# drscotthawley/signaltrain

Measured on AMD Instinct MI355X. Metric: audio-frames/sec (train step) comp_4c 8192-sample windows @ 1/2/4/8 GPUs, higher is better.
Workload: dtype f32; 1 GPU; comp_4c synthetic, 8192-sample windows, batch 256/GPU, fp32 (BASELINE configs[1]); window=8192, frames_per_window=25, global_batch=256, parallelism=dp1

## Files before the change

### signaltrain_amd/csrc/st_api.hip

```cpp
#include <hip/hip_runtime.h>
#include <stdarg.h>
#include <stdio.h>
#include <string.h>
#include <math.h>
#include <mutex>
#include <set>
#include <type_traits>
#include <utility>
#include "st_common.h"
#include "st_gemm.h"
#include "st_gemm_planes.h"
#include "st_gemm_tn.h"
#include "st_gemm16.h"
#include "st_misc.h"
#include "st_ae.h"
#include "st_ae_wide.h"
#include "st_ae_split.h"
#include "st_ae32.h"
#include "st_dp.h"
#include "st_feed.h"
#include "st_feed_files.h"
#include "st_feed_live.h"
#include "st_feed_stream.h"
#include "st_predict.h"
// ... 119 lines not shown
    ST_TRY(check_dims(d));
    L->total = param_offsets(d, L->offs);
    L->n_stft = L->offs[4];
    L->PG = (int)(L->offs[22] - L->offs[4]);
    for (int l = 0; l < 9; ++l) {
        L->go.w[l] = (int)(L->offs[4 + 2 * l] - L->offs[4]);
        L->go.b[l] = (int)(L->offs[5 + 2 * l] - L->offs[4]);
    }
    L->KP = st_kp_of(d->F);
    return ST_OK;
}

static int num_cus()
{
    static int n = 0;
    if (!n) { int dev = 0; (void)hipGetDevice(&dev); hipDeviceProp_t p; if (hipGetDeviceProperties(&p, dev) == hipSuccess) n = p.multiProcessorCount; if (n <= 0) n = 256; }
    return n;
}
extern "C" int st_set_debug(int v) { return v == 0 ? ST_OK : st_fail(ST_ERR_ARG, "st_set_debug(%d): the product library has no run-time ablations (build with -DST_*_ABLATE=bits)", v); }
static int g_dp_inline = 1;
static int g_ae_save = 1;
static int g_ae_split = -1;
static int g_ae32 = 1;
static int g_pl_bf16 = 0;
static int g_wg_split = 0;
static int g_pl_dgrad = 0;
static int g_pl_shape = 3;
static int g_g16 = 1;
static int g_g16_dma = 0;
static int g_nt128 = 1;
static int g_tn128 = 1;
static int g_tn_fm = 3;
static int g_g16_crop = 15;
static int g_frs_nt = 1;
static int g_xt = 0;
static const int NORM_E_PARTIALS = 32;
static const int NORM_E_MAX = 4096;
static int g_wide_direct = 1;
static int g_an_bk = 32;
static int g_bk = 16;
static int g_wg_mode = 0;
#define ST_TUNING_LIST(X) X(g_ae_split, -1) X(g_ae_save, 1) X(g_dp_inline, 1) X(g_pl_bf16, 0) X(g_wg_split, 0) X(g_pl_dgrad, 0) X(g_pl_shape, 3) X(g_g16, 1) X(g_g16_dma, 0) \
    X(g_nt128, 1) X(g_tn128, 1) X(g_frs_nt, 1) X(g_xt, 0) X(g_an_bk, 32) X(g_bk, 16) X(g_wg_mode, 0) X(g_ae32, 1) X(g_wide_direct, 1) X(g_tn_fm, 3) X(g_g16_crop, 15)
static const struct { int first, count; int* var; int value; int* also; } k_tuning_codes[] = {
    {16, 1, &g_an_bk, 16, &g_bk}, {32, 1, &g_an_bk, 32, &g_bk},
    {100, 1, &g_wg_mode, 0, nullptr}, {102, 1, &g_wg_mode, 2, nullptr},
    {7000, 2, &g_xt, 0, nullptr},
    {8000, 2, &g_ae_split, 0, nullptr}, {8002, 1, &g_ae_split, -1, nullptr},
    {8100, 2, &g_ae32, 0, nullptr},
    {8200, 3, &g_ae_save, 0, nullptr},
    {8300, 2, &g_dp_inline, 0, nullptr},
    {9000, 2, &g_frs_nt, 0, nullptr},
    {9100, 1, &g_pl_shape, 0, nullptr}, {9103, 1, &g_pl_shape, 3, nullptr},
    {9200, 2, &g_pl_dgrad, 0, nullptr},
    {9300, 2, &g_wg_split, 0, nullptr},
    {9400, 2, &g_pl_bf16, 0, nullptr},
    {9500, 2, &g_tn128, 0, nullptr}, {9580, 1, &g_tn128, 2, nullptr}, {9581, 1, &g_tn128, 1, nullptr},
    {9582, 1, &g_tn128, 3, nullptr},
    {9540, 4, &g_tn_fm, 0, nullptr},
    {9560, 16, &g_g16_crop, 0, nullptr},
    {9600, 2, &g_g16, 0, nullptr},
    {9690, 4, &g_g16_dma, 0, nullptr},
    {9950, 2, &g_nt128, 0, nullptr},
    {9970, 2, &g_wide_direct, 0, nullptr},
};
extern "C" int st_set_tuning(int code)
{
    for (const auto& t : k_tuning_codes)
        if (code >= t.first && code < t.first + t.count) { *t.var = t.value + (code - t.first); if (t.also) *t.also = *t.var; return ST_OK; }
    return st_fail(ST_ERR_ARG, "st_set_tuning(%d): no such code", code);
}
extern "C" int st_get_tuning(int* out, int n)
{
    int i = 0;
#define X(v_, d_) if (out && i < n) out[i] = v_; ++i;
    ST_TUNING_LIST(X)
#undef X
    return i;
}
extern "C" int st_tuning_defaults(int* out, int n)
{
    int i = 0;
#define X(v_, d_) if (out && i < n) out[i] = d_; ++i;
    ST_TUNING_LIST(X)
#undef X
    return i;
}
extern "C" int st_reset_tuning(void)
{
#define X(v_, d_) v_ = d_;
    ST_TUNING_LIST(X)
#undef X
    return ST_OK;
}
static inline int gemm_ht(int prec) { return (prec == ST_PREC_BF16 || prec == ST_PREC_BF16_ALL) ? 1 : ((prec == ST_PREC_F16 || prec == ST_PREC_F16_ALL) ? 2 : (prec == ST_PREC_F32X3 ? 3 : 0)); }
static inline int ae_ht(int prec) { return prec == ST_PREC_BF16_ALL ? 1 : (prec == ST_PREC_F16_ALL ? 2 : 0); }
static inline float loss_scale_of(const st_dims* d) { return d->loss_scale > 0.f ? d->loss_scale : 1.0f; }
static inline float reg_scale_of(const st_dims* d) { return (float)(2e-5 / 10.0) / ((float)d->B * (float)d->OT * (float)d->F); }
static inline float reg_coef_of(const st_dims* d) { return loss_scale_of(d) * (float)(2e-5 / 10.0) / ((float)d->B * (float)d->OT * (float)d->F); }
static inline float expfac_of(const st_dims* d) { return (float)(7.0 / d->F); }
static int ensure_dyn_lds(const void* fn, const char* name)
{
    static std::mutex mu; static std::set<std::pair<int, const void*>> done;
    int dev = 0; (void)hipGetDevice(&dev);
    std::lock_guard<std::mutex> lk(mu);
    if (done.count({dev, fn})) return ST_OK;
// ... 272 lines not shown
}

static stg::RowMap synth_live(const st_dims* d) { return stg::live_frames(d->OT, d->H, d->N, d->N, d->y); }
static int synth_live_rows(const st_dims* d) { return synth_live(d).rows(d->B); }

static double synth_crop_fraction(const st_dims* d)
{
    const stg::RowMap ms = synth_live(d);
    long live = 0;
    for (int t = ms.t_lo; t < ms.t_lo + ms.Tv; ++t) { int lo, hi; stg::ntw_live_taps(t, t, d->H, d->N, d->N, d->y, lo, hi); live += hi - lo; }
    return 1.0 - (double)live / ((double)ms.Tv * (double)d->N);
}
static inline bool fm_div_exact(int R, int B) { return R >= 0 && B >= 1 && (unsigned long long)(unsigned)R * (unsigned long long)(unsigned)B < (1ull << 32); }
extern "C" int st_fm_div_exact(int R, int B) { return fm_div_exact(R, B) ? 1 : 0; }
static bool use_nt128(const st_dims* d, int M, int Nc, int ncus = 0)
{
    if (!(g_nt128 && gemm_ht(d->prec) == 0 && d->N % 32 == 0 && (M + 127) / 128 <= 255 && fm_div_exact(M, d->B))) return false;
    if (ncus <= 0) ncus = num_cus();
    return ((M + 127) / 128) * ((Nc + 127) / 128) * 2 <= ncus || synth_crop_fraction(d) >= 0.10;
}
enum { GEMM_ANALYSIS = 0, GEMM_FRAMES = 1, GEMM_DGRAD = 2 };
enum { SGP_PADDED = 1,
       SGP_G16 = 2,
       SGP_SFOLDT = 4 };
enum { GF_FP32 = 0,
       GF_HALF = 1,
       GF_PLANES = 2,
       GF_G16 = 3 };
enum { GK_SMALL = 0,
       GK_NT128 = 1,
       GK_PLANES = 2,
       GK_NT16 = 3, GK_NT256 = 4 };
static bool use_planes(const st_dims* d) { return (gemm_ht(d->prec) == 3 || (gemm_ht(d->prec) == 1 && g_pl_bf16)) && d->N % 16 == 0 && st_kp_of(d->F) % 16 == 0; }
static int planes_of(const st_dims* d) { return gemm_ht(d->prec) == 3 ? 3 : 1; }
template <class F> static inline auto with_planes(int pl, F&& f) { return pl == 1 ? f(ic<1>{}) : f(ic<3>{}); }
static bool use_g16(const st_dims* d)
{
    const int ht = gemm_ht(d->prec);
    return g_g16 && (ht == 1 || ht == 2) && !g_pl_bf16 && d->N % 128 == 0 && num_cus() > 0;
}
static int stft_family(const st_dims* d, int which, int flags)
{
    if (flags & SGP_PADDED) {
        if ((flags & SGP_G16) && use_g16(d)) return GF_G16;
        if (use_planes(d) && (which != GEMM_DGRAD || g_pl_dgrad)) return GF_PLANES;
    }
    return gemm_ht(d->prec) == 0 ? GF_FP32 : GF_HALF;
}
struct GemmOps { const float *A, *B, *B2; const unsigned short *A16, *B16, *Bpl; float in_scale; };
struct GemmPlan {
    const st_dims* d; GemmOps o;
    int which, flags, family, form;
    int waves, bk, xt;
    bool transposed;
    stg::RowMap live;
    int R, M, Nc, K, ns;
    size_t slab;
    bool frame_major; int crop;
    stg::NTWork wk;
};
static GemmPlan stft_plan(const st_dims* d, int which, int flags, const GemmOps& o, int ncus = 0)
{
    const int KP = st_kp_of(d->F), N = d->N;
    const bool padded = (flags & SGP_PADDED) != 0;
    GemmPlan p; p.d = d; p.o = o; p.which = which; p.flags = flags;
    p.live = which == GEMM_ANALYSIS ? stg::live_frames(d->T, d->H, N, N, d->L)
                                    : synth_live(d);
    p.R = p.M = p.live.rows(d->B);
    p.Nc = which == GEMM_ANALYSIS ? 2 * d->F : which == GEMM_FRAMES ? N : KP; p.K = which == GEMM_FRAMES ? KP : N;
    const SynthTile t = which == GEMM_ANALYSIS ? SynthTile{4, 1} : synth_tile(p.R);
    p.waves = t.waves; p.ns = t.ns; p.slab = which == GEMM_ANALYSIS ? 0 : (size_t)d->B * d->OT * p.Nc;
    p.family = stft_family(d, which, flags);
    p.bk = p.xt = 0; p.transposed = false; p.frame_major = false; p.crop = 0; p.wk.n = 0;
    if (p.family == GF_G16) {
        const int dma = which == GEMM_ANALYSIS ? 1 : which == GEMM_DGRAD ? 2 : 0;
        p.form = ((g_g16_dma & dma) && N % 64 == 0 && N / 64 >= p.ns) ? GK_NT256 : GK_NT16; p.waves = 0;
        const bool crop = which == GEMM_FRAMES ? (g_g16_crop & 1) != 0 : which == GEMM_DGRAD && (g_g16_crop & 2) && !(g_g16_dma & 2);
        if (crop && fm_div_exact(p.R, d->B)) { p.frame_major = true; p.crop = which; }
    } else if (p.family == GF_PLANES) {
        p.form = GK_PLANES;
        if (which == GEMM_ANALYSIS && planes_of(d) == 3 && g_pl_shape == 3) p.waves = 8;
    } else {
        p.form = GK_SMALL;
        p.transposed = which == GEMM_FRAMES && (flags & SGP_SFOLDT) && g_frs_nt;
        const int cus = ncus > 0 ? ncus : num_cus();
        if ((which == GEMM_FRAMES ? p.transposed : which == GEMM_DGRAD && padded) && use_nt128(d, p.R, p.Nc, cus) &&
            (which == GEMM_FRAMES ? stg::ntw_frames(p.wk, p.live, d->B, d->H, N, N, d->y, KP, p.ns, cus)
                                  : stg::ntw_dgrad(p.wk, p.live, d->B, d->H, N, N, d->y, d->F, KP, p.ns, cus))) {
            p.form = GK_NT128; p.waves = 0; p.frame_major = true; p.crop = which;
        } else {
            p.wk.n = 0;
            if (p.family == GF_FP32) { p.bk = (which == GEMM_ANALYSIS && padded) ? g_an_bk : g_bk; p.xt = g_xt ? 1 : 0; }
        }
    }
    return p;
}
struct GemmOut { float *re, *im, *mag, *phs; const PolarWide* pw; float* C; };
static GemmOut slabs_at(float* C) { return GemmOut{nullptr, nullptr, nullptr, nullptr, nullptr, C}; }
static int stft_gemm(const GemmPlan& p, const GemmOut& out, void* stream)
{
    const st_dims* d = p.d; const GemmOps& o = p.o; hipStream_t s = st_stream(stream);
    const int KP = st_kp_of(d->F), N = d->N, R = p.R;
    const stg::RowMap rows = p.frame_major ? stg::frame_major(p.live, d->B) : p.live;
    auto g16 = [&](const stg::Rows16& ra, const stg::Rows16& rb, const auto& ep, const stg::Crop16* cr) {
        return with_ht16(gemm_ht(d->prec), [&](auto HT) {
            return p.form == GK_NT256 ? stg::launch16_nt256<HT()>(ra, rb, ep, p.M, p.Nc, p.K, p.ns, s) : stg::launch16_nt<HT()>(ra, rb, ep, p.M, p.Nc, p.K, p.ns, s, cr); }); };
    if (p.which == GEMM_ANALYSIS) {
        stg::PolarStore ep{out.re, out.im, out.mag, out.phs, R, d->F, rows};
        polar_wide_set(ep, out.pw);
        if (p.family == GF_G16)
            ST_TRY(g16(stg::rows16(o.A16, (unsigned)(d->L + 2 * N), (unsigned)d->H, p.live, R), stg::rows16_plain(o.B16, (unsigned)N, 2 * d->F), ep, nullptr));
        else if (!(p.flags & SGP_PADDED)) {
            stg::FramedNT<false> al{o.A, d->L, d->H, N, R, N, o.in_scale, p.live};
            ST_TRY(small_gemm<4>(d->prec, p.bk, p.xt != 0, al, stg::AnalysisW{o.B, o.B2, d->F, N}, ep, p.M, p.Nc, p.K, p.ns, s));
        } else {
            stg::FramedNT<true> al{o.A, d->L, d->H, N, R, N, 1.0f, p.live};
            if (p.family == GF_PLANES) {
                stg::ChunkP bl{o.Bpl, 2 * d->F};
                ST_TRY((planes_of(d) == 1 ? stg::launch_planes<4, 1>(al, bl, ep, p.M, p.Nc, p.K, p.ns, s) :
                        p.waves == 8 ? stg::launch_planes<8, 3>(al, bl, ep, p.M, p.Nc, p.K, p.ns, s) : stg::launch_planes<4, 3>(al, bl, ep, p.M, p.Nc, p.K, p.ns, s)));
            } else ST_TRY(small_gemm<4>(d->prec, p.bk, p.xt != 0, al, stg::AnalysisW{o.B, o.B2, d->F, N}, ep, p.M, p.Nc, p.K, p.ns, s));
        }
        ST_LAUNCHED("analysis_fwd");
        return ST_OK;
    }
    const bool frames = p.which == GEMM_FRAMES;
    const unsigned s_win = frames ? (unsigned)(d->OT * KP) : (unsigned)(d->y + 2 * N), s_frm = frames ? (unsigned)KP : (unsigned)d->H;
    auto small = [&](const auto& al, const auto& bl) {
        const stg::StoreC ep{out.C, R, p.Nc, p.Nc, p.slab, rows};
        return p.waves == 4 ? small_gemm<4>(d->prec, p.bk, p.xt != 0, al, bl, ep, p.M, p.Nc, p.K, p.ns, s) : small_gemm<2>(d->prec, p.bk, p.xt != 0, al, bl, ep, p.M, p.Nc, p.K, p.ns, s); };
    auto planes = [&](const auto& al) {
        const stg::StoreC ep{out.C, R, p.Nc, p.Nc, p.slab, rows}; const stg::ChunkP bl{o.Bpl, p.Nc};
        return with_planes(planes_of(d), [&](auto PL) {
            return p.waves == 4 ? stg::launch_planes<4, PL()>(al, bl, ep, p.M, p.Nc, p.K, p.ns, s) : stg::launch_planes<2, PL()>(al, bl, ep, p.M, p.Nc, p.K, p.ns, s); }); };
    if (p.family == GF_G16) {
        const stg::Rows16 ra = p.frame_major ? stg::rows16_frame_major(o.A16, s_win, s_frm, p.live, d->B, R) : stg::rows16(o.A16, s_win, s_frm, p.live, R);
        const stg::Crop16 cr{p.crop, d->B, d->H, N, N, d->y, p.live.t_lo, R, 1};
        ST_TRY(g16(ra, stg::rows16_plain(o.B16, (unsigned)p.K, p.Nc), stg::StoreC{out.C, R, p.Nc, p.Nc, p.slab, rows}, &cr));
    } else if (p.form == GK_NT128) {
        const stg::NTRows ra = stg::ntrows_frame_major(o.A, s_win, s_frm, p.live, d->B, R);
        const stg::NTRows rb = frames ? stg::NTRows{o.B2, (unsigned)KP, 0u, 0u, 1, 0, N} :
                               p.wk.col_h ? stg::NTRows{o.B, (unsigned)((KP / 2) * N), (unsigned)N, stg::rowmap_magic(d->F - 1), d->F - 1, 0, 2 * (d->F - 1)}
                                          : stg::NTRows{o.B, (unsigned)N, 0u, 0u, 1, 0, KP};
        ST_TRY(stg::launch_nt128(ra, rb, stg::StoreSlab{out.C, R, p.Nc, p.Nc, p.slab, rows}, p.wk, s));
    } else if (frames) {
        const stg::PlainNT al{o.A, R, KP, KP, p.live};
        if (p.family == GF_PLANES) ST_TRY(planes(al));
        else if (p.transposed) ST_TRY(small(al, stg::PlainNT{o.B2, N, KP, KP, stg::all_frames(1)}));
        else ST_TRY(small(al, stg::PlainTN{o.B, KP, N, N, stg::all_frames(1)}));
    } else {
        const stg::PlainNT bl{o.B, KP, N, N, stg::all_frames(1)};
        if (!(p.flags & SGP_PADDED)) ST_TRY(small(stg::FramedNT<false>{o.A, d->y, d->H, N, R, N, 1.0f, p.live}, bl));
        else {
            const stg::FramedNT<true> al{o.A, d->y, d->H, N, R, N, 1.0f, p.live};
            if (p.family == GF_PLANES) ST_TRY(planes(al)); else ST_TRY(small(al, bl));
        }
    }
    ST_LAUNCHED(frames ? "synthesis_frames" : "synthesis_dgrad");
    return ST_OK;
}
extern "C" int st_analysis_fwd(const st_dims* d, const float* x, const float* Wr, const float* Wi, float in_scale,
                               float* re, float* im, float* mag, float* phs, void* stream)
{
    ST_TRY(check_dims(d)); ST_REQ(x && Wr && Wi, "st_analysis_fwd: null input");
    const GemmPlan p = stft_plan(d, GEMM_ANALYSIS, 0, GemmOps{x, Wr, Wi, nullptr, nullptr, nullptr, in_scale});
    ST_TRY(stft_gemm(p, GemmOut{re, im, mag, phs, nullptr, nullptr}, stream));
    if (p.live.Tv < d->T) {
        hipLaunchKernelGGL(stm::zero_dead_frames_kernel, dim3(d->B * (d->T - p.live.Tv)), dim3(256), 0, st_stream(stream),
                           re, im, mag, phs, d->T, d->F, p.live.t_lo, p.live.Tv);
        ST_LAUNCHED("zero_dead_frames");
    }
    return ST_OK;
}
extern "C" int st_synthesis_frames(const st_dims* d, const float* AA, const float* Sfold, float* frs, void* stream)
// ... 1947 lines not shown
```

### signaltrain_amd/csrc/st_gemm.h

```cpp
#pragma once
#include "st_common.h"

static int ensure_dyn_lds(const void* fn, const char* name);
namespace stg {

constexpr int BK = 32;
constexpr int BN = 96;
constexpr int NJ = BN / 32;
constexpr int PK = BK + 4;

struct RowMap {
    int Tv, t_lo, T; unsigned magic;
    int fm;
    __host__ __device__ int rows(int B) const { return B * Tv; }
    __device__ void split(int r, int& b, int& t) const {
        if (fm) {
            const int q = magic ? (int)__umulhi((unsigned)r, magic) : r;
            b = r - (int)__umul24((unsigned)q, (unsigned)fm);
            t = t_lo + q;
            return;
        }
        b = magic ? (int)__umulhi((unsigned)r, magic) : r;
        t = t_lo + (r - (int)__umul24((unsigned)b, (unsigned)Tv));
    }
    __device__ int full(int r) const { int b, t; split(r, b, t); return (int)__umul24((unsigned)b, (unsigned)T) + t; }
};
static inline unsigned rowmap_magic(int Tv) { return Tv > 1 ? (unsigned)(((unsigned long long)1 << 32) / (unsigned)Tv) + 1u : 0u; }
static inline RowMap live_frames(int T, int H, int N, int pad, int Ls)
{
    int lo = 0, hi = T - 1;
    while (lo < T && H * lo - pad + N <= 0) ++lo;
    while (hi >= lo && H * hi - pad >= Ls) --hi;
    RowMap m; m.t_lo = lo; m.Tv = hi - lo + 1; m.T = T; m.fm = 0;
    if (m.Tv <= 0) { m.Tv = T; m.t_lo = 0; }
    m.magic = rowmap_magic(m.Tv);
    return m;
}
static inline RowMap all_frames(int T) { RowMap m; m.Tv = T; m.t_lo = 0; m.T = T; m.fm = 0; m.magic = rowmap_magic(T); return m; }
static inline RowMap frame_major(RowMap m, int B) { m.fm = B; m.magic = B > 1 ? rowmap_magic(B) : 0u; return m; }

__device__ __forceinline__ float4 ldg128(const float* __restrict__ base, const unsigned elem)
{
    return *reinterpret_cast<const float4*>(reinterpret_cast<const char*>(base) + (size_t)(elem << 2));
}

struct Src { const float* p; bool ok; };

struct TNParams { const float* base; unsigned magic, S1, S2; int Tv, t_lo, clampR, klim, collim; };

struct RowState {
    const float* p;
    unsigned o;
    int lo, hi;
};

template <bool PADDED>
struct FramedNT {
    static constexpr bool kTN = false;
    static constexpr bool kCheck = !PADDED;
    static constexpr bool kOff = true;
    const float* sig; int Ls, H, pad, R, Kw; float scale; RowMap map;
    __device__ const float* dummy() const { return sig; }
    __device__ RowState row_state(int r) const {
        RowState s; s.p = sig; s.o = 0; s.lo = 0; s.hi = 0;
        if (PADDED) {
            int b, t; map.split(r < R ? r : 0, b, t);
            s.o = __umul24((unsigned)b, (unsigned)(Ls + 2 * pad)) + __umul24((unsigned)H, (unsigned)t);
            s.p = sig + s.o;
            s.hi = Kw;
        } else if (r < R) {
            int b, t; map.split(r, b, t);
            const int start = H * t - pad;
            s.o = __umul24((unsigned)b, (unsigned)Ls) + (unsigned)start;
            s.p = sig + (size_t)b * Ls + start;
            s.lo = start < 0 ? -start : 0;
            s.hi = (Ls - start) < Kw ? (Ls - start) : Kw;
            if (s.hi < s.lo) s.hi = s.lo;
        }
        return s;
    }
    __device__ Src src(const RowState& s, int k) const { return Src{s.p + k, PADDED || (k >= s.lo && k < s.hi)}; }
    __device__ float4 post(float4 v) const {
        if (!PADDED) { v.x *= scale; v.y *= scale; v.z *= scale; v.w *= scale; }
        return v;
    }
};

template <bool PADDED>
struct FramedTN {
    static constexpr bool kTN = true;
    static constexpr bool kCheck = !PADDED;
    static constexpr bool kOff = true;
    const float* sig; int Ls, H, pad, R, Kw; float scale; RowMap map;
    __device__ const float* dummy() const { return sig; }
    __device__ Src src(int r, int n) const {
        if (PADDED) {
            int b, t; map.split(r < R ? r : 0, b, t);
            return Src{sig + (size_t)b * (Ls + 2 * pad) + H * t + n, true};
        }
        Src s{sig, false};
        if (r < R && n < Kw) {
            int b, t; map.split(r, b, t);
            const int pos = H * t - pad + n;
            s.ok = pos >= 0 && pos < Ls;
            s.p = sig + (size_t)b * Ls + pos;
        }
        return s;
    }
    __device__ unsigned off(int r, int n, bool& ok) const {
        int b, t;
        map.split(r < R ? r : 0, b, t);
        if (PADDED) {
            ok = true;
            return __umul24((unsigned)b, (unsigned)(Ls + 2 * pad)) + __umul24((unsigned)H, (unsigned)t) + (unsigned)n;
        }
        const int pos = H * t - pad + n;
        ok = r < R && n < Kw && pos >= 0 && pos < Ls;
        return ok ? __umul24((unsigned)b, (unsigned)Ls) + (unsigned)pos : 0u;
    }
    __device__ float4 post(float4 v) const {
        if (!PADDED) { v.x *= scale; v.y *= scale; v.z *= scale; v.w *= scale; }
        return v;
    }
    static constexpr bool kParams = PADDED;
    __device__ TNParams tn_params() const { return TNParams{sig, map.magic, (unsigned)(Ls + 2 * pad), (unsigned)H, map.Tv, map.t_lo, R, 0x7fffffff, 0x7fffffff}; }
};

struct PlainNT {
    static constexpr bool kTN = false;
    static constexpr bool kCheck = false;
    static constexpr bool kOff = true;
    const float* base; int R, ld, K; RowMap map;
    __device__ const float* dummy() const { return base; }
    __device__ RowState row_state(int r) const {
        RowState s; s.lo = 0; s.hi = K;
        s.o = __umul24((unsigned)map.full(r < R ? r : 0), (unsigned)ld);
        s.p = base + s.o;
        return s;
    }
    __device__ Src src(const RowState& s, int k) const { return Src{s.p + k, true}; }
    __device__ float4 post(float4 v) const { return v; }
};

struct PlainTN {
    static constexpr bool kTN = true;
    static constexpr bool kCheck = true;
    static constexpr bool kOff = true;
    const float* base; int K, ld, cols; RowMap map;
    __device__ const float* dummy() const { return base; }
    __device__ Src src(int k, int c) const {
        const bool ok = k < K && c < cols;
        return Src{base + (size_t)(ok ? map.full(k) : 0) * ld + c, ok};
    }
    __device__ unsigned off(int k, int c, bool& ok) const {
        ok = k < K && c < cols;
        return ok ? __umul24((unsigned)map.full(k), (unsigned)ld) + (unsigned)c : 0u;
    }
    __device__ float4 post(float4 v) const { return v; }
    static constexpr bool kParams = true;
    __device__ TNParams tn_params() const { return TNParams{base, map.magic, (unsigned)(map.T * ld), (unsigned)ld, map.Tv, map.t_lo, K, K, cols}; }
};

struct AnalysisW {
    static constexpr bool kTN = false;
    static constexpr bool kCheck = false;
    static constexpr bool kOff = false;
    const float* Wr; const float* Wi; int F, N;
    __device__ const float* dummy() const { return Wr; }
    __device__ RowState row_state(int j) const {
        const int bin = j >> 1;
        RowState s; s.lo = 0; s.hi = N; s.o = 0;
        s.p = ((j & 1) ? Wi : Wr) + (size_t)(bin < F ? bin : 0) * N;
        return s;
    }
    __device__ Src src(const RowState& s, int k) const { return Src{s.p + k, true}; }
    __device__ float4 post(float4 v) const { return v; }
};

#ifndef ST_XCD_SWIZZLE
#define ST_XCD_SWIZZLE 1
#endif
__device__ __forceinline__ void xcd_tile(int& bx, int& by, int& bz, const int nz_ = 0)
{
    bx = blockIdx.x; by = blockIdx.y; bz = blockIdx.z;
#if ST_XCD_SWIZZLE
    const int nx = gridDim.x, ny = gridDim.y, nz = nz_ > 0 ? nz_ : (int)gridDim.z;
    const int T = nx * ny * nz;
    if (T < 16) return;
    const int L = bx + nx * (by + ny * bz);
    const int j = L & 7, q = T >> 3, r = T & 7;
    const int Lp = j * q + (j < r ? j : r) + (L >> 3);
    bz = Lp / (nx * ny);
    const int rem = Lp - bz * (nx * ny);
    if (ny > nx) { bx = rem / ny; by = rem - bx * ny; }
    else { by = rem / nx; bx = rem - by * nx; }
#endif
}

__device__ __forceinline__ void xcd_tile_2d(int& bx, int& by, int& bz)
{
    bx = blockIdx.x; by = blockIdx.y; bz = 0;
#if ST_XCD_SWIZZLE
    const int nx = gridDim.x, ny = gridDim.y;
    const int T = nx * ny;
    if (T < 64 || nx < 2 || ny < 4) { xcd_tile(bx, by, bz); return; }
    const int L = bx + nx * by;
    const int j = L & 7, q = T >> 3, r = T & 7;
    int p = j * q + (j < r ? j : r) + (L >> 3);
#pragma unroll
    for (int blk = 0; blk < 8; ++blk) {
        const int rb = blk >> 1, cb = blk & 1;
        const int r0 = (rb * ny) >> 2, r1 = ((rb + 1) * ny) >> 2, c0 = (cb * nx) >> 1, c1 = ((cb + 1) * nx) >> 1;
        const int sz = (r1 - r0) * (c1 - c0);
        if (p < sz) { const int rr = p / (c1 - c0); by = r0 + rr; bx = c0 + (p - rr * (c1 - c0)); return; }
        p -= sz;
    }
#endif
}

__device__ __forceinline__ int d_row(int i, int lane) { return (i & 3) + 8 * (i >> 2) + 4 * (lane >> 5); }

struct StoreC {
    float* out; int M, Nc, ld; size_t slab; RowMap map;
    __device__ StoreC slab_shifted(int dz) const { StoreC e = *this; e.out += (size_t)dz * slab; return e; }
    template <int NJX>
    __device__ void operator()(int m0, int n0, const f32x16 (&acc)[NJX]) const {
        const int lane = threadIdx.x & 63;
        int tbx, tby, tbz; xcd_tile(tbx, tby, tbz);
// ... 19 lines not shown
        const int lane = threadIdx.x & 63;
        float bv[NJ];
#pragma unroll
        for (int j = 0; j < NJ; ++j) { const int col = n0 + 32 * j + (lane & 31); bv[j] = (bias && col < Nc) ? bias[col] : 0.f; }
#pragma unroll
        for (int i = 0; i < 16; ++i) {
            const int row = m0 + d_row(i, lane);
            if (row < M) {
#pragma unroll
                for (int j = 0; j < NJ; ++j) {
                    const int col = n0 + 32 * j + (lane & 31);
                    if (col < Nc) out[(size_t)row * ld + col] = acc[j][i] + bv[j];
                }
            }
        }
    }
};

struct PolarStore {
    float* re; float* im; float* mag; float* phs; int R, F; RowMap map;
    float* Vm = nullptr; float* Vp = nullptr; int FP = 0; unsigned RV = 0;
    template <int NJX>
    __device__ void operator()(int m0, int n0, const f32x16 (&acc)[NJX]) const {
        const int lane = threadIdx.x & 63;
        const bool odd = lane & 1;
#pragma unroll
        for (int i = 0; i < 16; i += 2) {
            const int row = m0 + d_row(i + (odd ? 1 : 0), lane);
            int wb = 0, wt = 0; map.split(row < R ? row : 0, wb, wt);
            const size_t rbase = (size_t)((int)__umul24((unsigned)wb, (unsigned)map.T) + wt) * F;
            const size_t vbase = (size_t)wt * RV + (size_t)wb * FP;
#pragma unroll
            for (int j = 0; j < NJX; ++j) {
                const int bin = (n0 + 32 * j + (lane & 31)) >> 1;
                const float v0 = acc[j][i], v1 = acc[j][i + 1];
                const float got = __shfl_xor(odd ? v0 : v1, 1);
                const float vr = odd ? got : v0, vi = odd ? v1 : got;
                if (row < R && bin < F) {
                    const size_t idx = rbase + bin;
                    if (re) re[idx] = vr;
                    if (im) im[idx] = vi;
                    if (mag || phs || Vm) {
                        const float mg = __builtin_amdgcn_sqrtf(vr * vr + vi * vi), ph = st_atan2f(vi, vr + 1e-7f);
                        if (mag) mag[idx] = mg;
                        if (phs) phs[idx] = ph;
                        if (Vm) { Vm[vbase + bin] = mg; Vp[vbase + bin] = ph; }
                    }
                }
            }
        }
    }
};

template <class E> constexpr bool kPolarEpi = false;
template <> constexpr bool kPolarEpi<PolarStore> = true;
template <class L, class = void> struct has_tn_params { static constexpr bool value = false; };
template <class L> struct has_tn_params<L, decltype((void)L::kParams)> { static constexpr bool value = L::kParams; };

#ifndef ST_GEMM_ABLATE
#define ST_GEMM_ABLATE 0
#endif
#define ST_DBG(bit_) (ST_GEMM_ABLATE & (bit_))
__device__ __forceinline__ int xq_slot(const int row, const int q) { (void)q; return (row & ~3) | ((row + (row >> 3)) & 3); }
template <int WAVES_M, int BKT, bool XT, class AL, class BL, class EPI>
__global__ void __launch_bounds__(WAVES_M * 64)
gemm_kernel(const AL al, const BL bl, const EPI epi, const int K, const int ksplit)
{
    constexpr int BM = 32 * WAVES_M, NT = 64 * WAVES_M;
    constexpr int PKT = BKT + 4;
    constexpr bool A_T = AL::kTN && XT, A_K = AL::kTN && !XT;
    constexpr bool B_T = BL::kTN && XT, B_K = BL::kTN && !XT;
    constexpr int LDA = A_K ? BM + 4 : PKT;
    constexpr int LDB = B_K ? BN + 4 : PKT;
    constexpr int A_SZ = A_T ? BKT * BM : (A_K ? BKT * LDA : BM * LDA);
    constexpr int B_SZ = B_T ? BKT * BN : (B_K ? BKT * LDB : BN * LDB);
    constexpr int KQ = BKT / 4;
    constexpr int A_N = A_T ? (BM / 4) * KQ : BM * KQ;
    constexpr int B_N = B_T ? (BN / 4) * KQ : BN * KQ;
    constexpr int A_LD = A_T ? 4 : 1, B_LD = B_T ? 4 : 1;
    constexpr int A_IT = (A_N + NT - 1) / NT, B_IT = (B_N + NT - 1) / NT;
    constexpr int HK = BKT / 2;
    __shared__ __attribute__((aligned(16))) float As[2 * A_SZ];
    __shared__ __attribute__((aligned(16))) float Bs[2 * B_SZ];

    const int tid = threadIdx.x, lane = tid & 63, wave = tid >> 6;
    int tbx, tby, tbz;
    if constexpr (kPolarEpi<EPI>) xcd_tile_2d(tbx, tby, tbz); else xcd_tile(tbx, tby, tbz);
    const int m_blk = tby * BM, n_blk = tbx * BN;
    const int k_begin = tbz * ksplit;
    const int k_end = (k_begin + ksplit < K) ? k_begin + ksplit : K;

    int a_i[A_IT], a_k[A_IT], a_l[A_IT], b_i[B_IT], b_k[B_IT], b_l[B_IT];
    bool a_v[A_IT], b_v[B_IT];
    RowState a_st[AL::kTN ? 1 : A_IT], b_st[BL::kTN ? 1 : B_IT];
#pragma unroll
    for (int p = 0; p < A_IT; ++p) {
        const int idx = tid + NT * p;
        a_v[p] = idx < A_N;
        const int id = a_v[p] ? idx : 0;
        if constexpr (A_T) { a_i[p] = (id % (BM / 4)) * 4; a_k[p] = (id / (BM / 4)) * 4; a_l[p] = 0; }
        else if constexpr (A_K) { a_i[p] = (id % (BM / 4)) * 4; a_k[p] = id / (BM / 4); a_l[p] = a_k[p] * LDA + a_i[p]; }
        else { a_i[p] = id / KQ; a_k[p] = (id % KQ) * 4; a_l[p] = a_i[p] * LDA + a_k[p]; a_st[p] = al.row_state(m_blk + a_i[p]); }
    }
#pragma unroll
    for (int p = 0; p < B_IT; ++p) {
        const int idx = (B_T ? NT - 1 - tid : tid) + NT * p;
        b_v[p] = idx < B_N;
        const int id = b_v[p] ? idx : 0;
        if constexpr (B_T) { b_i[p] = (id % (BN / 4)) * 4; b_k[p] = (id / (BN / 4)) * 4; b_l[p] = 0; }
        else if constexpr (B_K) { b_i[p] = (id % (BN / 4)) * 4; b_k[p] = id / (BN / 4); b_l[p] = b_k[p] * LDB + b_i[p]; }
        else { b_i[p] = id / KQ; b_k[p] = (id % KQ) * 4; b_l[p] = b_i[p] * LDB + b_k[p]; b_st[p] = bl.row_state(n_blk + b_i[p]); }
    }

    constexpr bool UNI = A_T && B_T && (A_N + B_N <= NT) && A_IT == 1 && B_IT == 1 && has_tn_params<AL>::value && has_tn_params<BL>::value;
    const bool u_isA = tid < A_N;
// ... 131 lines not shown
#pragma unroll
            for (int j = 0; j < NJ; ++j)
#pragma unroll
                for (int q = 0; q < HK / 4; ++q) { const int kq = (HK / 4) * h + q; b_xq[j][q] = (kq * BN + xq_slot(32 * j + l31, kq)) * 4; }
        }
        for (int kt = k_begin; kt < k_end; kt += BKT) {
            const bool more = kt + BKT < k_end;
            if (!ST_DBG(1)) gload(more ? kt + BKT : kt);
            __builtin_amdgcn_sched_barrier(0);
            const float* as = As + cur * A_SZ + a_off;
            const float* bs = Bs + cur * B_SZ + b_off;
            if (!ST_DBG(4)) {
                float af[HK], bf[NJ][HK];
                if constexpr (!A_K) {
#pragma unroll
                    for (int q = 0; q < HK / 4; ++q) {
                        const float4 v = *reinterpret_cast<const float4*>(A_T ? as + a_xq[A_T ? q : 0] : as + 4 * q);
                        af[4 * q] = v.x; af[4 * q + 1] = v.y; af[4 * q + 2] = v.z; af[4 * q + 3] = v.w;
                    }
                }
                if constexpr (!B_K) {
#pragma unroll
                    for (int j = 0; j < NJ; ++j)
#pragma unroll
                        for (int q = 0; q < HK / 4; ++q) {
                            const float4 v = *reinterpret_cast<const float4*>(B_T ? bs + b_xq[B_T ? j : 0][B_T ? q : 0] : bs + 32 * j * LDB + 4 * q);
                            bf[j][4 * q] = v.x; bf[j][4 * q + 1] = v.y; bf[j][4 * q + 2] = v.z; bf[j][4 * q + 3] = v.w;
                        }
                }
#pragma unroll
                for (int kk = 0; kk < HK; ++kk) {
                    float a, b[NJ];
                    if constexpr (A_K) a = as[kk * LDA]; else a = af[kk];
#pragma unroll
                    for (int j = 0; j < NJ; ++j) { if constexpr (B_K) b[j] = bs[kk * LDB + 32 * j]; else b[j] = bf[j][kk]; }
#pragma unroll
                    for (int j = 0; j < NJ; ++j) acc[j] = __builtin_amdgcn_mfma_f32_32x32x2f32(a, b[j], acc[j], 0, 0, 0);
                }
                if constexpr (A_K && B_K) {
                    __builtin_amdgcn_sched_group_barrier(0x100, 4, 0);
#pragma unroll
                    for (int kk = 0; kk < HK; ++kk) {
                        __builtin_amdgcn_sched_group_barrier(0x100, 2, 0);
                        __builtin_amdgcn_sched_group_barrier(0x008, NJ, 0);
                    }
                }
            }
            __builtin_amdgcn_sched_barrier(0);
            if (!ST_DBG(1)) lstore(cur ^ 1);
            if (!ST_DBG(2)) __syncthreads();
            cur ^= 1;
        }
    }
    epi(m_blk + wave * 32, n_blk, acc);
}

typedef __bf16 st_bf16x8 __attribute__((ext_vector_type(8)));
typedef _Float16 st_f16x8 __attribute__((ext_vector_type(8)));
__device__ __forceinline__ unsigned st_pack_bf16(float a, float b)
{
    unsigned r; asm volatile("v_cvt_pk_bf16_f32 %0, %1, %2" : "=v"(r) : "v"(a), "v"(b)); return r;
}
__device__ __forceinline__ unsigned st_pack_f16(float a, float b)
{
    unsigned r; asm volatile("v_cvt_pk_f16_f32 %0, %1, %2" : "=v"(r) : "v"(a), "v"(b)); return r;
}
template <int HT> __device__ __forceinline__ unsigned st_pack_h(float a, float b) { if constexpr (HT == 2) return st_pack_f16(a, b); else return st_pack_bf16(a, b); }

__device__ __forceinline__ float st_bf16_lo(unsigned p) { return __uint_as_float(p << 16); }
__device__ __forceinline__ float st_bf16_hi(unsigned p) { return __uint_as_float(p & 0xffff0000u); }
__device__ __forceinline__ unsigned st_cvt_pk_bf16(const float a, const float b)
{
    typedef __bf16 bf16x2_t __attribute__((ext_vector_type(2)));
    typedef float f32x2_t __attribute__((ext_vector_type(2)));
    union { bf16x2_t h; unsigned u; } r; r.h = __builtin_convertvector((f32x2_t){a, b}, bf16x2_t); return r.u;
}
__device__ __forceinline__ void st_split3(const float x, const float y, const float z, const float w, uint2 (&pl)[3])
{
    float r[4] = {x, y, z, w};
#pragma unroll
    for (int p = 0; p < 3; ++p) {
        pl[p] = make_uint2(st_cvt_pk_bf16(r[0], r[1]), st_cvt_pk_bf16(r[2], r[3]));
        if (p < 2) { r[0] -= st_bf16_lo(pl[p].x); r[1] -= st_bf16_hi(pl[p].x); r[2] -= st_bf16_lo(pl[p].y); r[3] -= st_bf16_hi(pl[p].y); }
    }
}
#ifndef ST_SPLIT_VALU_PER_MFMA
#define ST_SPLIT_VALU_PER_MFMA 5
#endif
template <int WAVES_M, int HT, int PL, int BKH, class AL, class BL, class EPI>
__device__ __forceinline__ void
gemm_half_body(const AL& al, const BL& bl, const EPI& epi, const int K, const int ksplit, const int tbx, const int tby, const int tbz)
{
    static_assert(PL == 1 || (PL == 3 && HT == 1), "the split needs the fp32 exponent range: bfloat16 planes only");
    constexpr int BM = 32 * WAVES_M, NT = 64 * WAVES_M;
    constexpr int LD = BKH + 8;
    constexpr int A_SZ = BM * LD, B_SZ = BN * LD;
    constexpr int KQ = BKH / 4;
    constexpr int A_N = AL::kTN ? (BM / 4) * KQ : BM * KQ;
    constexpr int B_N = BL::kTN ? (BN / 4) * KQ : BN * KQ;
    constexpr int A_IT = (A_N + NT - 1) / NT, B_IT = (B_N + NT - 1) / NT;
    constexpr int A_LDS = AL::kTN ? 4 : 1, B_LDS = BL::kTN ? 4 : 1;
    extern __shared__ __attribute__((aligned(16))) unsigned short half_lds[];
    unsigned short* const As = half_lds;
    unsigned short* const Bs = half_lds + 2 * PL * A_SZ;
    unsigned short* const dump = half_lds + 2 * PL * (A_SZ + B_SZ) + 4 * threadIdx.x;

// ... 263 lines not shown
__global__ void __launch_bounds__(WAVES_M * 64)
gemm_half_kernel(const AL al, const BL bl, const EPI epi, const int K, const int ksplit)
{
    int tbx, tby, tbz; xcd_tile(tbx, tby, tbz);
    gemm_half_body<WAVES_M, HT, PL, BKH>(al, bl, epi, K, ksplit, tbx, tby, tbz);
}
template <int WAVES_M, int HT, int PL, int BKH, class AL, class BL, class EPI>
__global__ void __launch_bounds__(WAVES_M * 64)
gemm_half_pair_kernel(const AL al0, const BL bl0, const EPI epi0, const AL al1, const BL bl1, const EPI epi1, const int K, const int ksplit, const int nzh)
{
    int tbx, tby, tbz; xcd_tile(tbx, tby, tbz);
    if (tbz < nzh) gemm_half_body<WAVES_M, HT, PL, BKH>(al0, bl0, epi0, K, ksplit, tbx, tby, tbz);
    else gemm_half_body<WAVES_M, HT, PL, BKH>(al1, bl1, epi1, K, ksplit, tbx, tby, tbz - nzh);
}

template <int WAVES_M, int HT = 1, int PL = 1, int BKH = (PL == 3 ? 16 : 32), class AL, class BL, class EPI>
static inline int launch_half_pair(const AL& al0, const BL& bl0, const EPI& epi0, const AL& al1, const BL& bl1, const EPI& epi1,
                                   int M, int Nc, int K, int nsplit, hipStream_t s)
{
    constexpr int BM = 32 * WAVES_M;
    constexpr size_t lds = ((size_t)2 * PL * (BM + BN) * (BKH + 8) + (PL == 3 ? 4 * 64 * WAVES_M : 0)) * sizeof(unsigned short);
    int ksplit = K;
    if (nsplit > 1) ksplit = st_round_up((K + nsplit - 1) / nsplit, 32);
    const int nzh = nsplit > 1 ? nsplit : 1;
    dim3 grid((Nc + BN - 1) / BN, (M + BM - 1) / BM, 2 * nzh);
    if (lds > 65536) { const int rc = ::ensure_dyn_lds((const void*)gemm_half_pair_kernel<WAVES_M, HT, PL, BKH, AL, BL, EPI>, "gemm_half_pair_kernel"); if (rc) return rc; }
    hipLaunchKernelGGL((gemm_half_pair_kernel<WAVES_M, HT, PL, BKH, AL, BL, EPI>), grid, dim3(WAVES_M * 64), lds, s, al0, bl0, epi0, al1, bl1, epi1, K, ksplit, nzh);
    return 0;
}

template <int WAVES_M, int HT = 1, int PL = 1, int BKH = (PL == 3 ? 16 : 32), class AL, class BL, class EPI>
static inline int launch_half(const AL& al, const BL& bl, const EPI& epi, int M, int Nc, int K, int nsplit, hipStream_t s)
{
    constexpr int BM = 32 * WAVES_M;
    constexpr size_t lds = ((size_t)2 * PL * (BM + BN) * (BKH + 8) + (PL == 3 ? 4 * 64 * WAVES_M : 0)) * sizeof(unsigned short);
    int ksplit = K;
    if (nsplit > 1) ksplit = st_round_up((K + nsplit - 1) / nsplit, 32);
    dim3 grid((Nc + BN - 1) / BN, (M + BM - 1) / BM, nsplit > 1 ? nsplit : 1);
    if (lds > 65536) { const int rc = ::ensure_dyn_lds((const void*)gemm_half_kernel<WAVES_M, HT, PL, BKH, AL, BL, EPI>, "gemm_half_kernel"); if (rc) return rc; }
    hipLaunchKernelGGL((gemm_half_kernel<WAVES_M, HT, PL, BKH, AL, BL, EPI>), grid, dim3(WAVES_M * 64), lds, s, al, bl, epi, K, ksplit);
    return 0;
}

template <int WAVES_M, int BKT, bool XT = false, class AL, class BL, class EPI>
static inline void launch(const AL& al, const BL& bl, const EPI& epi, int M, int Nc, int K, int nsplit, hipStream_t s)
{
    constexpr int BM = 32 * WAVES_M;
    int ksplit = K;
    if (nsplit > 1) ksplit = st_round_up((K + nsplit - 1) / nsplit, BK);
    dim3 grid((Nc + BN - 1) / BN, (M + BM - 1) / BM, nsplit > 1 ? nsplit : 1);
    hipLaunchKernelGGL((gemm_kernel<WAVES_M, BKT, XT, AL, BL, EPI>), grid, dim3(WAVES_M * 64), 0, s, al, bl, epi, K, ksplit);
}

}
```

Before: 11.38 million frames/s.

## Add trimmed NT fp32 analysis GEMM with buffer loads and specialized polar epilogue

```diff
diff --git a/signaltrain_amd/csrc/st_api.hip b/signaltrain_amd/csrc/st_api.hip
--- a/signaltrain_amd/csrc/st_api.hip
+++ b/signaltrain_amd/csrc/st_api.hip
@@ -195,6 +195,7 @@
     {8300, 2, &g_dp_inline, 0, nullptr},
     {9000, 2, &g_frs_nt, 0, nullptr},
     {9100, 1, &g_pl_shape, 0, nullptr}, {9103, 1, &g_pl_shape, 3, nullptr},
+    {9330, 1, &g_an_bk, -32, nullptr},
     {9200, 2, &g_pl_dgrad, 0, nullptr},
     {9300, 2, &g_wg_split, 0, nullptr},
     {9400, 2, &g_pl_bf16, 0, nullptr},
@@ -573,6 +574,7 @@
     const st_dims* d; GemmOps o;
     int which, flags, family, form;
     int waves, bk, xt;
+    bool trim;
     bool transposed;
     stg::RowMap live;
     int R, M, Nc, K, ns;
@@ -592,7 +594,7 @@
     const SynthTile t = which == GEMM_ANALYSIS ? SynthTile{4, 1} : synth_tile(p.R);
     p.waves = t.waves; p.ns = t.ns; p.slab = which == GEMM_ANALYSIS ? 0 : (size_t)d->B * d->OT * p.Nc;
     p.family = stft_family(d, which, flags);
-    p.bk = p.xt = 0; p.transposed = false; p.frame_major = false; p.crop = 0; p.wk.n = 0;
+    p.bk = p.xt = 0; p.trim = false; p.transposed = false; p.frame_major = false; p.crop = 0; p.wk.n = 0;
     if (p.family == GF_G16) {
         const int dma = which == GEMM_ANALYSIS ? 1 : which == GEMM_DGRAD ? 2 : 0;
         p.form = ((g_g16_dma & dma) && N % 64 == 0 && N / 64 >= p.ns) ? GK_NT256 : GK_NT16; p.waves = 0;
@@ -611,13 +613,39 @@
             p.form = GK_NT128; p.waves = 0; p.frame_major = true; p.crop = which;
         } else {
             p.wk.n = 0;
-            if (p.family == GF_FP32) { p.bk = (which == GEMM_ANALYSIS && padded) ? g_an_bk : g_bk; p.xt = g_xt ? 1 : 0; }
+            if (p.family == GF_FP32) { p.bk = (which == GEMM_ANALYSIS && padded) ? (g_an_bk < 0 ? -g_an_bk : g_an_bk) : g_bk; p.xt = g_xt ? 1 : 0; }
+            p.trim = p.family == GF_FP32 && which == GEMM_ANALYSIS && padded && g_an_bk == 32 && !p.xt && p.ns == 1 && p.K % 32 == 0;
         }
     }
     return p;
 }
 struct GemmOut { float *re, *im, *mag, *phs; const PolarWide* pw; float* C; };
 static GemmOut slabs_at(float* C) { return GemmOut{nullptr, nullptr, nullptr, nullptr, nullptr, C}; }
+static int analysis_trim(const GemmPlan& p, const stg::FramedNT<true>& al, const stg::PolarStore& ep, hipStream_t s, bool* done)
+{
+    const st_dims* d = p.d; const int N = d->N;
+    *done = false;
+    if ((ep.re != nullptr) != (ep.im != nullptr) || (ep.mag != nullptr) != (ep.phs != nullptr) || (ep.Vm != nullptr) != (ep.Vp != nullptr)) return ST_OK;
+    const int set = (ep.re ? stg::POLAR_REIM : 0) | (ep.mag ? stg::POLAR_ROWS : 0) | (ep.Vm ? stg::POLAR_WIDE : 0);
+    if (!set) return ST_OK;
+    const float* const W0 = p.o.B < p.o.B2 ? p.o.B : p.o.B2;
+    const size_t oR = (size_t)(p.o.B - W0), oI = (size_t)(p.o.B2 - W0), wspan = (oR > oI ? oR : oI) + (size_t)d->F * N;
+    const size_t xspan = (size_t)d->B * ((size_t)d->L + 2 * (size_t)N);
+    if (wspan >= ((size_t)1 << 30) || xspan >= ((size_t)1 << 30)) return ST_OK;
+    ST_REQ((size_t)d->B * d->T * d->F < ((size_t)1 << 30) && (!ep.Vm || (size_t)d->T * ep.RV < ((size_t)1 << 30)),
+           "analysis forward: batch too large for the polar epilogue's 32-bit element offsets (B=%d)", d->B);
+    const stg::AnalysisW32 bl{W0, (unsigned)oR, (unsigned)oI, d->F, N};
+    auto go = [&](auto SET) {
+        const stg::PolarStoreSet<SET()> es{ep.re, ep.im, ep.mag, ep.phs, ep.R, ep.F, ep.map, ep.Vm, ep.Vp, ep.FP, ep.RV};
+        stg::launch_nt<4, 32>(al, bl, es, p.M, p.Nc, p.K, (unsigned)(xspan * sizeof(float)), (unsigned)(wspan * sizeof(float)), s);
+    };
+    switch (set) {
+    case 1: go(ic<1>{}); break; case 2: go(ic<2>{}); break; case 3: go(ic<3>{}); break; case 4: go(ic<4>{}); break;
+    case 5: go(ic<5>{}); break; case 6: go(ic<6>{}); break; default: go(ic<7>{}); break;
+    }
+    *done = true;
+    return ST_OK;
+}
 static int stft_gemm(const GemmPlan& p, const GemmOut& out, void* stream)
 {
     const st_dims* d = p.d; const GemmOps& o = p.o; hipStream_t s = st_stream(stream);
@@ -640,7 +668,11 @@
                 stg::ChunkP bl{o.Bpl, 2 * d->F};
                 ST_TRY((planes_of(d) == 1 ? stg::launch_planes<4, 1>(al, bl, ep, p.M, p.Nc, p.K, p.ns, s) :
                         p.waves == 8 ? stg::launch_planes<8, 3>(al, bl, ep, p.M, p.Nc, p.K, p.ns, s) : stg::launch_planes<4, 3>(al, bl, ep, p.M, p.Nc, p.K, p.ns, s)));
-            } else ST_TRY(small_gemm<4>(d->prec, p.bk, p.xt != 0, al, stg::AnalysisW{o.B, o.B2, d->F, N}, ep, p.M, p.Nc, p.K, p.ns, s));
+            } else {
+                bool done = false;
+                if (p.trim) ST_TRY(analysis_trim(p, al, ep, s, &done));
+                if (!done) ST_TRY(small_gemm<4>(d->prec, p.bk, p.xt != 0, al, stg::AnalysisW{o.B, o.B2, d->F, N}, ep, p.M, p.Nc, p.K, p.ns, s));
+            }
         }
         ST_LAUNCHED("analysis_fwd");
         return ST_OK;
diff --git a/signaltrain_amd/csrc/st_gemm.h b/signaltrain_amd/csrc/st_gemm.h
--- a/signaltrain_amd/csrc/st_gemm.h
+++ b/signaltrain_amd/csrc/st_gemm.h
@@ -22,6 +22,12 @@
         }
         b = magic ? (int)__umulhi((unsigned)r, magic) : r;
         t = t_lo + (r - (int)__umul24((unsigned)b, (unsigned)Tv));
+    }
+    __device__ void split_flat(int r, int& b, int& t) const {
+        const unsigned q = __umulhi((unsigned)r, magic) + ((unsigned)r & (magic ? 0u : ~0u));
+        const unsigned rem = (unsigned)r - __umul24(q, (unsigned)(fm ? fm : Tv));
+        b = (int)(fm ? rem : q);
+        t = t_lo + (int)(fm ? q : rem);
     }
     __device__ int full(int r) const { int b, t; split(r, b, t); return (int)__umul24((unsigned)b, (unsigned)T) + t; }
 };
@@ -84,6 +90,7 @@
         if (!PADDED) { v.x *= scale; v.y *= scale; v.z *= scale; v.w *= scale; }
         return v;
     }
+    __device__ unsigned row_off(int r) const { static_assert(PADDED, "row_off: the padded copy only"); return row_state(r).o; }
 };
 
 template <bool PADDED>
@@ -174,6 +181,15 @@
         return s;
     }
     __device__ Src src(const RowState& s, int k) const { return Src{s.p + k, true}; }
+    __device__ float4 post(float4 v) const { return v; }
+};
+struct AnalysisW32 {
+    const float* W0; unsigned oR, oI; int F, N;
+    __device__ const float* dummy() const { return W0; }
+    __device__ unsigned row_off(int j) const {
+        const int bin = j >> 1;
+        return ((j & 1) ? oI : oR) + (unsigned)(bin < F ? bin : 0) * (unsigned)N;
+    }
     __device__ float4 post(float4 v) const { return v; }
 };
 
@@ -299,15 +315,67 @@
     }
 };
 
-template <class E> constexpr bool kPolarEpi = false;
-template <> constexpr bool kPolarEpi<PolarStore> = true;
-template <class L, class = void> struct has_tn_params { static constexpr bool value = false; };
-template <class L> struct has_tn_params<L, decltype((void)L::kParams)> { static constexpr bool value = L::kParams; };
-
+enum { POLAR_REIM = 1, POLAR_ROWS = 2, POLAR_WIDE = 4 };
+__device__ __forceinline__ void stg32(float* __restrict__ base, const unsigned byte_off, const int imm, const float v)
+{
+    *reinterpret_cast<float*>(reinterpret_cast<char*>(base) + (size_t)byte_off + imm) = v;
+}
+__device__ __forceinline__ void st_keep(const float v) { asm volatile("" : : "v"(v)); }
 #ifndef ST_GEMM_ABLATE
 #define ST_GEMM_ABLATE 0
 #endif
+template <int SET>
+struct PolarStoreSet {
+    float* re; float* im; float* mag; float* phs; int R, F; RowMap map;
+    float* Vm; float* Vp; int FP; unsigned RV;
+    template <bool MASK, int NJX>
+    __device__ __forceinline__ void rows(const int m0, const int n0, const f32x16 (&acc)[NJX]) const {
+        const int lane = threadIdx.x & 63;
+        const bool odd = lane & 1;
+        const int bin0 = (n0 + (lane & 31)) >> 1;
+#pragma unroll
+        for (int i = 0; i < 16; i += 2) {
+            const int row = m0 + d_row(i + (odd ? 1 : 0), lane);
+            int wb = 0, wt = 0; map.split_flat(MASK ? (row < R ? row : 0) : row, wb, wt);
+            const unsigned rb = ((__umul24((unsigned)wb, (unsigned)map.T) + (unsigned)wt) * (unsigned)F + (unsigned)bin0) << 2;
+            const unsigned vb = ((unsigned)wt * RV + __umul24((unsigned)wb, (unsigned)FP) + (unsigned)bin0) << 2;
+#pragma unroll
+            for (int j = 0; j < NJX; ++j) {
+                const float v0 = acc[j][i], v1 = acc[j][i + 1];
+                const float got = __shfl_xor(odd ? v0 : v1, 1);
+                const float vr = odd ? got : v0, vi = odd ? v1 : got;
+                if (!MASK || (row < R && bin0 + 16 * j < F)) {
+                    float mg = vr, ph = vi;
+                    if (!(ST_GEMM_ABLATE & 16) && (SET & (POLAR_ROWS | POLAR_WIDE))) { mg = __builtin_amdgcn_sqrtf(vr * vr + vi * vi); ph = st_atan2f(vi, vr + 1e-7f); }
+                    if (ST_GEMM_ABLATE & 8) { st_keep(vr); st_keep(vi); st_keep(mg); st_keep(ph); continue; }
+                    if (SET & POLAR_REIM) { stg32(re, rb, 64 * j, vr); stg32(im, rb, 64 * j, vi); }
+                    if (SET & POLAR_ROWS) { stg32(mag, rb, 64 * j, mg); stg32(phs, rb, 64 * j, ph); }
+                    if (SET & POLAR_WIDE) { stg32(Vm, vb, 64 * j, mg); stg32(Vp, vb, 64 * j, ph); }
+                }
+            }
+        }
+    }
+    template <int NJX>
+    __device__ void operator()(const int m0, const int n0, const f32x16 (&acc)[NJX]) const {
+        if (m0 + 32 <= R && n0 + 32 * NJX <= 2 * F) rows<false>(m0, n0, acc); else rows<true>(m0, n0, acc);
+    }
+};
+
+template <class E> constexpr bool kPolarEpi = false;
+template <> constexpr bool kPolarEpi<PolarStore> = true;
+template <int SET> constexpr bool kPolarEpi<PolarStoreSet<SET>> = true;
+template <class L, class = void> struct has_tn_params { static constexpr bool value = false; };
+template <class L> struct has_tn_params<L, decltype((void)L::kParams)> { static constexpr bool value = L::kParams; };
+
 #define ST_DBG(bit_) (ST_GEMM_ABLATE & (bit_))
+template <int NJX>
+__device__ __forceinline__ void keep_acc(const f32x16 (&acc)[NJX])
+{
+#pragma unroll
+    for (int j = 0; j < NJX; ++j)
+#pragma unroll
+        for (int i = 0; i < 16; ++i) st_keep(acc[j][i]);
+}
 __device__ __forceinline__ int xq_slot(const int row, const int q) { (void)q; return (row & ~3) | ((row + (row >> 3)) & 3); }
 template <int WAVES_M, int BKT, bool XT, class AL, class BL, class EPI>
 __global__ void __launch_bounds__(WAVES_M * 64)
@@ -545,6 +613,102 @@
             cur ^= 1;
         }
     }
+    if (ST_DBG(32) && kPolarEpi<EPI>) { keep_acc(acc); return; }
+    epi(m_blk + wave * 32, n_blk, acc);
+}
+
+template <int WAVES_M, int BKT, class AL, class BL, class EPI>
+__global__ void __launch_bounds__(WAVES_M * 64)
+gemm_nt_kernel(const AL al, const BL bl, const EPI epi, const int K, const unsigned a_bytes, const unsigned b_bytes)
+{
+    constexpr int BM = 32 * WAVES_M, NT = 64 * WAVES_M;
+    constexpr int PKT = BKT + 4, KQ = BKT / 4, HK = BKT / 2;
+    constexpr int A_SZ = BM * PKT, B_SZ = BN * PKT;
+    constexpr int RP = NT / KQ;
+    static_assert((BM * KQ) % NT == 0 && (BN * KQ) % NT == 0, "gemm_nt_kernel: whole passes only");
+    constexpr int A_IT = BM * KQ / NT, B_IT = BN * KQ / NT;
+    __shared__ __attribute__((aligned(16))) float As[2 * A_SZ];
+    __shared__ __attribute__((aligned(16))) float Bs[2 * B_SZ];
+
+    const int tid = threadIdx.x, lane = tid & 63, wave = tid >> 6;
+    int tbx, tby, tbz;
+    if constexpr (kPolarEpi<EPI>) xcd_tile_2d(tbx, tby, tbz); else xcd_tile(tbx, tby, tbz);
+    const int m_blk = tby * BM, n_blk = tbx * BN;
+
+    const int it_row = tid / KQ, it_k = (tid % KQ) * 4;
+    unsigned a_o[A_IT], b_o[B_IT];
+#pragma unroll
+    for (int p = 0; p < A_IT; ++p) a_o[p] = (al.row_off(m_blk + it_row + RP * p) + (unsigned)it_k) << 2;
+#pragma unroll
+    for (int p = 0; p < B_IT; ++p) b_o[p] = (bl.row_off(n_blk + it_row + RP * p) + (unsigned)it_k) << 2;
+    const int st_l = it_row * PKT + it_k;
+    const int h = lane >> 5, l31 = lane & 31;
+    const float* const a_fr = As + (wave * 32 + l31) * PKT + HK * h;
+    const float* const b_fr = Bs + l31 * PKT + HK * h;
+
+    const __amdgpu_buffer_rsrc_t a_rs = __builtin_amdgcn_make_buffer_rsrc(const_cast<float*>(al.dummy()), 0, a_bytes, 0x00020000);
+    const __amdgpu_buffer_rsrc_t b_rs = __builtin_amdgcn_make_buffer_rsrc(const_cast<float*>(bl.dummy()), 0, b_bytes, 0x00020000);
+    float4 ra[A_IT], rb[B_IT];
+    auto gload = [&](const int kt) {
+#pragma unroll
+        for (int p = 0; p < A_IT; ++p) ra[p] = __builtin_bit_cast(float4, __builtin_amdgcn_raw_buffer_load_b128(a_rs, a_o[p], kt * 4, 0));
+#pragma unroll
+        for (int p = 0; p < B_IT; ++p) rb[p] = __builtin_bit_cast(float4, __builtin_amdgcn_raw_buffer_load_b128(b_rs, b_o[p], kt * 4, 0));
+    };
+    auto lstore = [&](const int stage) {
+#pragma unroll
+        for (int p = 0; p < A_IT; ++p) *reinterpret_cast<float4*>(As + stage * A_SZ + st_l + RP * PKT * p) = al.post(ra[p]);
+#pragma unroll
+        for (int p = 0; p < B_IT; ++p) *reinterpret_cast<float4*>(Bs + stage * B_SZ + st_l + RP * PKT * p) = bl.post(rb[p]);
+    };
+
+    f32x16 acc[NJ];
+#pragma unroll
+    for (int j = 0; j < NJ; ++j)
+#pragma unroll
+        for (int i = 0; i < 16; ++i) acc[j][i] = 0.f;
+
+    auto body = [&](const int stage, const int next) {
+        if (!ST_DBG(1)) gload(next);
+        __builtin_amdgcn_sched_barrier(0);
+        if (!ST_DBG(4)) {
+            const float* const as = a_fr + stage * A_SZ;
+            const float* const bs = b_fr + stage * B_SZ;
+            float af[HK], bf[NJ][HK];
+#pragma unroll
+            for (int q = 0; q < HK / 4; ++q) {
+                const float4 v = *reinterpret_cast<const float4*>(as + 4 * q);
+                af[4 * q] = v.x; af[4 * q + 1] = v.y; af[4 * q + 2] = v.z; af[4 * q + 3] = v.w;
+            }
+#pragma unroll
+            for (int j = 0; j < NJ; ++j)
+#pragma unroll
+                for (int q = 0; q < HK / 4; ++q) {
+                    const float4 v = *reinterpret_cast<const float4*>(bs + 32 * j * PKT + 4 * q);
+                    bf[j][4 * q] = v.x; bf[j][4 * q + 1] = v.y; bf[j][4 * q + 2] = v.z; bf[j][4 * q + 3] = v.w;
+                }
+#pragma unroll
+            for (int kk = 0; kk < HK; ++kk)
+#pragma unroll
+                for (int j = 0; j < NJ; ++j) acc[j] = __builtin_amdgcn_mfma_f32_32x32x2f32(af[kk], bf[j][kk], acc[j], 0, 0, 0);
+        }
+        __builtin_amdgcn_sched_barrier(0);
+        if (!ST_DBG(1)) lstore(stage ^ 1);
+        if (!ST_DBG(2)) __syncthreads();
+    };
+
+    if (K > 0) {
+        gload(0);
+        lstore(0);
+        __syncthreads();
+        int kt = 0;
+        for (; kt + 2 * BKT <= K; kt += 2 * BKT) {
+            body(0, kt + BKT);
+            body(1, kt + 2 * BKT < K ? kt + 2 * BKT : kt + BKT);
+        }
+        if (kt < K) body(0, kt);
+    }
+    if (ST_DBG(32)) { keep_acc(acc); return; }
     epi(m_blk + wave * 32, n_blk, acc);
 }
 
@@ -914,4 +1078,11 @@
     hipLaunchKernelGGL((gemm_kernel<WAVES_M, BKT, XT, AL, BL, EPI>), grid, dim3(WAVES_M * 64), 0, s, al, bl, epi, K, ksplit);
 }
 
-}
+template <int WAVES_M, int BKT, class AL, class BL, class EPI>
+static inline void launch_nt(const AL& al, const BL& bl, const EPI& epi, int M, int Nc, int K, unsigned a_bytes, unsigned b_bytes, hipStream_t s)
+{
+    constexpr int BM = 32 * WAVES_M;
+    hipLaunchKernelGGL((gemm_nt_kernel<WAVES_M, BKT, AL, BL, EPI>), dim3((Nc + BN - 1) / BN, (M + BM - 1) / BM, 1), dim3(WAVES_M * 64), 0, s, al, bl, epi, K, a_bytes, b_bytes);
+}
+
+}
```

After: 11.41 million frames/s, median of 6. No clear change (+0.2%).
